# MarbleHE/ABC

Measured on AMD Instinct MI355X. Metric: homomorphic mul+relin/sec, CKKS N=2^14, higher is better.
Workload: dtype u64 (transforms: exact integer arithmetic in f64); 1 GPU; CKKS N=16384, 4 data limbs {50,40,40,40} + special 50-bit prime, ct x ct multiply + relinearize; total_batch=8192, batch_rank0=8192

## Files before the change

### abc_amd/csrc/abc_context.hip

```cpp
#include <cstdlib>
#include <cstring>
#include <mutex>

#include "../../include/abc_hip.h"
#include <dlfcn.h>

#include "abc_context.hpp"
#include "abc_host_math.hpp"

namespace abc {

static thread_local std::string g_err;
void set_error(const std::string &msg) { g_err = msg; }

static bool env_on(const char *name) {
  const char *e = std::getenv(name);
  return e && !(e[0] == '0' && e[1] == 0);
}
void read_switches(abc_hip_ctx *c) {
  abc_hip_ctx::Switches s;
  s.no_fused = env_on("ABC_HIP_NO_FUSED");
  s.no_split = env_on("ABC_HIP_NO_SPLIT");
  s.no_split4 = env_on("ABC_HIP_NO_SPLIT4");
  s.no_isplit = env_on("ABC_HIP_NO_ISPLIT");
  s.no_gsplit = env_on("ABC_HIP_NO_GSPLIT");
  s.no_bsplit = env_on("ABC_HIP_NO_BSPLIT");
  s.no_mixed = env_on("ABC_HIP_NO_MIXED");
  s.no_pack = env_on("ABC_HIP_NO_PACK");
  s.no_key_twin = env_on("ABC_HIP_NO_KEY_TWIN");
  s.no_bmul = env_on("ABC_HIP_NO_BMUL");
  s.no_special8x2 = env_on("ABC_HIP_NO_SPECIAL8X2");
  s.no_bmul_mid = env_on("ABC_HIP_NO_BMUL_MID");
  s.no_finish_lds = env_on("ABC_HIP_NO_FINISH_LDS");
  s.no_iks = env_on("ABC_HIP_NO_IKS");
  s.no_bmul_r6 = env_on("ABC_HIP_NO_BMUL_R6");
  s.no_lean_front = env_on("ABC_HIP_NO_LEAN_FRONT");
  s.no_tensor_intt = env_on("ABC_HIP_NO_TENSOR_INTT");
  s.no_galois_fusion = env_on("ABC_HIP_NO_GALOIS_FUSION");
  if (const char *e = std::getenv("ABC_HIP_CHUNK")) s.chunk = (size_t)std::atol(e);
  if (const char *e = std::getenv("ABC_HIP_FEW_LIMBS")) s.few_limbs = (size_t)std::atol(e);
  if (const char *e = std::getenv("ABC_HIP_LEAN_LIMIT")) s.lean_limit = (size_t)std::atol(e);
  if (const char *e = std::getenv("ABC_HIP_PASS0_TARGET_LIMIT")) s.pass0_target_limit = (size_t)std::atol(e);
  if (const char *e = std::getenv("ABC_HIP_BFV_SCRATCH_MB")) s.bfv_scratch_mb = (size_t)std::atol(e);
  if (const char *e = std::getenv("ABC_HIP_LANE_OFFSET_US")) s.lane_offset_us = (unsigned)std::atoi(e);
  if (const char *e = std::getenv("ABC_HIP_LANES")) {
    s.lanes = std::atoi(e);
    if (s.lanes < 1) s.lanes = 1;
    if (s.lanes > abc_hip_ctx::kMaxLanes) s.lanes = abc_hip_ctx::kMaxLanes;
  }
  c->sw = s;
}

static bool capturing(abc_hip_ctx *c) {
  hipStreamCaptureStatus st = hipStreamCaptureStatusNone;
  if (hipStreamIsCapturing(c->stream, &st) != hipSuccess) return false;
  return st != hipStreamCaptureStatusNone;
}

static int trim_cache(abc_hip_ctx *c) {
  std::lock_guard<std::mutex> lock(c->alloc_mu);
  if (c->free_blocks.empty()) return 0;
  ABC_HIP_CHECK(hipStreamSynchronize(c->stream));
  for (auto &kv : c->free_blocks)
    for (void *p : kv.second) {
      c->block_size.erase(p);
      (void)hipFree(p);
    }
  c->free_blocks.clear();
  c->cached_bytes = 0;
  return 0;
}
static hipError_t malloc_retry(abc_hip_ctx *c, void **p, size_t bytes) {
  hipError_t e = hipMalloc(p, bytes);
  if (e == hipSuccess) return e;
  (void)hipGetLastError();
  if (trim_cache(c)) return e;
  return hipMalloc(p, bytes);
}

void retire_buffer(abc_hip_ctx *c, void *p, uint64_t born) {
  if (!p) return;
  abc_hip_ctx::Held h{p, {}};
  for (auto &kv : c->live_graphs)
    if (kv.second > born) h.graphs.push_back(kv.first);
  if (h.graphs.empty()) {
    (void)hipFree(p);
    return;
  }
  c->held.push_back(std::move(h));
}

int ensure_workspace(abc_hip_ctx *c, size_t bytes) {
  if (bytes <= c->ws_bytes) return 0;
  if (capturing(c)) { set_error("scratch would grow during graph capture: run the sequence once eagerly first"); return 1; }
  if (c->ws) {
    ABC_HIP_CHECK(hipStreamSynchronize(c->stream));
    retire_buffer(c, c->ws, c->ws_born);
    c->ws = nullptr;
    c->ws_bytes = 0;
  }
  size_t want = bytes + bytes / 8;
  ABC_HIP_CHECK(malloc_retry(c, &c->ws, want));
  c->ws_bytes = want;
  c->ws_born = c->graph_seq;
  return 0;
}

int ensure_aux(abc_hip_ctx *c, int which, size_t bytes) {
  if (bytes <= c->aux_bytes[which]) return 0;
  if (capturing(c)) { set_error("scratch would grow during graph capture: run the sequence once eagerly first"); return 1; }
  if (c->aux[which]) {
    ABC_HIP_CHECK(hipStreamSynchronize(c->stream));
    retire_buffer(c, c->aux[which], c->aux_born[which]);
    c->aux[which] = nullptr;
    c->aux_bytes[which] = 0;
  }
  ABC_HIP_CHECK(malloc_retry(c, &c->aux[which], bytes));
  c->aux_bytes[which] = bytes;
  c->aux_born[which] = c->graph_seq;
  return 0;
}
// ... 422 lines not shown
  static const uint64_t p1024[] = {0x7e00001ull};
  static const uint64_t p2048[] = {0x3fffffff000001ull};
  static const uint64_t p4096[] = {0xffffee001ull, 0xffffc4001ull, 0x1ffffe0001ull};
  static const uint64_t p8192[] = {0x7fffffd8001ull, 0x7fffffc8001ull, 0xfffffffc001ull, 0xffffff6c001ull, 0xfffffebc001ull};
  static const uint64_t p16384[] = {0xfffffffd8001ull,  0xfffffffa0001ull,  0xfffffff00001ull,  0x1fffffff68001ull, 0x1fffffff50001ull,
                                    0x1ffffffee8001ull, 0x1ffffffea0001ull, 0x1ffffffe88001ull, 0x1ffffffe48001ull};
  static const uint64_t p32768[] = {0x7fffffffe90001ull, 0x7fffffffbf0001ull, 0x7fffffffbd0001ull, 0x7fffffffba0001ull,
                                    0x7fffffffaa0001ull, 0x7fffffffa50001ull, 0x7fffffff9f0001ull, 0x7fffffff7e0001ull,
                                    0x7fffffff770001ull, 0x7fffffff380001ull, 0x7fffffff330001ull, 0x7fffffff2d0001ull,
                                    0x7fffffff170001ull, 0x7fffffff150001ull, 0x7ffffffef00001ull, 0xfffffffff70001ull};
  const uint64_t *src = nullptr;
  int cnt = 0;
  switch (n) {
    case 1024: src = p1024; cnt = 1; break;
    case 2048: src = p2048; cnt = 1; break;
    case 4096: src = p4096; cnt = 3; break;
    case 8192: src = p8192; cnt = 5; break;
    case 16384: src = p16384; cnt = 9; break;
    case 32768: src = p32768; cnt = 16; break;
    default: set_error("no default BFV coefficient modulus for this ring degree"); return -1;
  }
  for (int i = 0; i < cnt; i++) out[i] = src[i];
  return cnt;
}

uint64_t abc_hip_plain_modulus_batching(size_t n, int bits) {
  try {
    return host::ntt_primes(n, bits, 1)[0];
  } catch (const std::exception &e) {
    set_error(e.what());
    return 0;
  }
}

int abc_hip_create_primes(size_t n, const int *bit_sizes, int count, uint64_t *out) {
  try {
    std::map<int, std::vector<uint64_t>> table;
    for (int i = 0; i < count; i++) table[bit_sizes[i]];
    for (auto &kv : table) {
      size_t need = 0;
      for (int i = 0; i < count; i++) need += (bit_sizes[i] == kv.first);
      kv.second = host::ntt_primes(n, kv.first, need);
    }
    for (int i = 0; i < count; i++) {
      auto &v = table[bit_sizes[i]];
      out[i] = v.back();
      v.pop_back();
    }
    return 0;
  } catch (const std::exception &e) {
    set_error(e.what());
    return 1;
  }
}

int abc_hip_ctx_create(int scheme, int logn, const uint64_t *primes, int nprimes, uint64_t plain_modulus, int device,
                       abc_hip_ctx **out) {
  if (!out) { set_error("null output pointer"); return 1; }
  *out = nullptr;
  if (scheme != ABC_HIP_SCHEME_BFV && scheme != ABC_HIP_SCHEME_CKKS) { set_error("unknown scheme"); return 1; }
  if (logn < 10 || logn > 16) { set_error("logn must be in 10..16"); return 1; }
  if (nprimes < 2 || nprimes > kMaxLimbs) { set_error("need 2..16 primes (data limbs + special prime)"); return 1; }
  const uint64_t two_n = 2ull << logn;
  for (int i = 0; i < nprimes; i++) {
    if (primes[i] >> 60 || !host::is_prime(primes[i]) || primes[i] % two_n != 1) {
      set_error("coefficient modulus primes must be < 2^60, prime and = 1 mod 2N");
      return 1;
    }
    for (int j = 0; j < i; j++)
      if (primes[j] == primes[i]) { set_error("coefficient modulus primes must be distinct"); return 1; }
  }
  if (scheme == ABC_HIP_SCHEME_BFV) {
    if (!host::is_prime(plain_modulus) || plain_modulus % two_n != 1 || plain_modulus >> 32) {
      set_error("plain modulus must be a prime = 1 mod 2N (batching) below 2^32");
      return 1;
    }
  }
  int ndev = 0;
  if (hipGetDeviceCount(&ndev) != hipSuccess || ndev <= 0) { set_error("no HIP device available"); return 1; }
  if (device < 0 || device >= ndev) { set_error("device index out of range"); return 1; }
  if (hipSetDevice(device) != hipSuccess) { set_error("hipSetDevice failed"); return 1; }
  abc_hip_ctx *c = new abc_hip_ctx();
  c->scheme = scheme; c->logn = logn; c->n = 1 << logn; c->K = nprimes; c->L = nprimes - 1; c->device = device;
  c->primes.assign(primes, primes + nprimes);
  c->t = (scheme == ABC_HIP_SCHEME_BFV) ? plain_modulus : 0;
  int rc = 1;
  try {
    rc = build_context(c);
  } catch (const std::exception &e) {
    set_error(e.what());
  }
  if (!rc && hipStreamCreateWithFlags(&c->own_stream, hipStreamNonBlocking) != hipSuccess) {
    set_error("hipStreamCreate failed");
    rc = 1;
  }
  if (!rc) c->stream = c->own_stream;
  if (!rc && (hipEventCreate(&c->ev0) != hipSuccess || hipEventCreate(&c->ev1) != hipSuccess ||
              hipEventCreateWithFlags(&c->lane_fork, hipEventDisableTiming) != hipSuccess)) {
    set_error("hipEventCreate failed");
    rc = 1;
  }
  int mask_mod = 0;
  if (const char *e = std::getenv("ABC_HIP_CU_MASK")) mask_mod = std::atoi(e);
  for (int i = 0; !rc && i < abc_hip_ctx::kMaxLanes; i++) {
    hipError_t se;
    if (mask_mod >= 2) {
      uint32_t mask[8];
      for (int w = 0; w < 8; w++) {
        mask[w] = 0;
        for (int b = 0; b < 32; b++)
          if (((w * 32 + b) % mask_mod) == (i % mask_mod)) mask[w] |= 1u << b;
      }
      se = hipExtStreamCreateWithCUMask(&c->lane[i], 8, mask);
    } else {
      se = hipStreamCreateWithFlags(&c->lane[i], hipStreamNonBlocking);
    }
    if (hipEventCreateWithFlags(&c->lane_join[i], hipEventDisableTiming) != hipSuccess || se != hipSuccess) {
      set_error("lane stream / event creation failed");
      rc = 1;
    }
  }
  if (!rc && !env_on("ABC_HIP_SYNC_ALLOC")) {
    c->cache_alloc = true;
    size_t free_b = 0, total_b = 0;
    if (hipMemGetInfo(&free_b, &total_b) == hipSuccess) c->cache_cap = total_b / 4;
  }
  if (rc) { abc_hip_ctx_destroy(c); return 1; }
  *out = c;
  return 0;
}

void abc_hip_ctx_destroy(abc_hip_ctx *c) {
  if (!c) return;
  (void)hipSetDevice(c->device);
  (void)hipDeviceSynchronize();
  (void)hipFree(c->d_mods); (void)hipFree(c->d_tw); (void)hipFree(c->d_ftw); (void)hipFree(c->d_cst); (void)hipFree(c->d_cstf);
  (void)hipFree(c->d_slot_map);
  (void)hipFree(c->d_ckks_codec);
  drop_key_twins(c, nullptr);
  (void)hipFree(c->d_sk); (void)hipFree(c->d_pk); (void)hipFree(c->d_relin);
  for (auto &kv : c->d_galois) (void)hipFree(kv.second);
  (void)hipFree(c->ws);
  for (void *p : c->aux) (void)hipFree(p);
  for (auto &h : c->held) (void)hipFree(h.p);
  for (auto &kv : c->block_size) (void)hipFree(kv.first);
  if (c->own_stream) (void)hipStreamDestroy(c->own_stream);
  if (c->ev0) (void)hipEventDestroy(c->ev0);
  if (c->ev1) (void)hipEventDestroy(c->ev1);
  if (c->lane_fork) (void)hipEventDestroy(c->lane_fork);
  for (int i = 0; i < abc_hip_ctx::kMaxLanes; i++) {
    if (c->lane_join[i]) (void)hipEventDestroy(c->lane_join[i]);
    if (c->lane[i]) (void)hipStreamDestroy(c->lane[i]);
  }
  delete c;
}

int abc_hip_ctx_info(const abc_hip_ctx *c, int what) {
  if (!c) return -1;
  switch (what) {
    case 0: return c->scheme;
    case 1: return c->logn;
    case 2: return c->K;
    case 3: return c->L;
    case 4: return c->device;
    case 5: return c->nBsk;
    case 6: return (int)c->held.size();
// ... 471 lines not shown
```

### abc_amd/csrc/abc_context.hpp

```cpp
#pragma once

#include <hip/hip_runtime.h>

#include <map>
#include <mutex>
#include <unordered_map>
#include <string>
#include <vector>

#include "abc_modarith.hpp"
#include "abc_ntt.hpp"

namespace abc {

constexpr int kMaxLimbs = 16;

struct LimbMap {
  int id[kMaxLimbs + 1];
};

struct DevConst {
  u64 inv_special[kMaxLimbs], inv_special_s[kMaxLimbs];
  u64 inv_qlast[kMaxLimbs][kMaxLimbs], inv_qlast_s[kMaxLimbs][kMaxLimbs];
  u64 special_mod_q[kMaxLimbs], special_mod_q_s[kMaxLimbs];
  double inv_special_c[kMaxLimbs], inv_special_cq[kMaxLimbs];
  double special_c[kMaxLimbs], special_cq[kMaxLimbs];
  double inv_qlast_c[kMaxLimbs][kMaxLimbs], inv_qlast_cq[kMaxLimbs][kMaxLimbs];
  u64 q_mod_t, upper_half_threshold, t;
  u64 coeff_div_plain[kMaxLimbs], upper_half_increment[kMaxLimbs];
  int nq, nB, nBsk, pad_;
  u64 mtilde_mod_q[kMaxLimbs];
  u64 inv_punct_q[kMaxLimbs];
  u64 q_to_bsk[kMaxLimbs][kMaxLimbs];
  u64 q_to_mtilde[kMaxLimbs];
  u64 neg_inv_q_mod_mtilde;
  u64 q_mod_bsk[kMaxLimbs], inv_mtilde_mod_bsk[kMaxLimbs], inv_q_mod_bsk[kMaxLimbs];
  u64 inv_punct_B[kMaxLimbs];
  u64 B_to_q[kMaxLimbs][kMaxLimbs];
  u64 B_to_msk[kMaxLimbs];
  u64 inv_B_mod_msk, B_mod_q[kMaxLimbs];
  u64 t_mod_q[kMaxLimbs], t_mod_bsk[kMaxLimbs];
  u64 ext_q[kMaxLimbs], ext_q_s[kMaxLimbs];
  u64 flr_q[kMaxLimbs], flr_q_s[kMaxLimbs];
  u64 tinvq_bsk[kMaxLimbs], tinvq_bsk_s[kMaxLimbs];
  u64 inv_q_mod_bsk_s[kMaxLimbs], inv_mtilde_mod_bsk_s[kMaxLimbs], inv_punct_B_s[kMaxLimbs];
  u64 inv_B_mod_msk_s, B_mod_q_s[kMaxLimbs];
  u64 dec_q[kMaxLimbs], dec_q_s[kMaxLimbs];
  u64 q_to_bsk_s[kMaxLimbs][kMaxLimbs], B_to_q_s[kMaxLimbs][kMaxLimbs], B_to_msk_s[kMaxLimbs], q_mod_bsk_s[kMaxLimbs];
  u64 tgamma_mod_q[kMaxLimbs], q_to_t[kMaxLimbs], q_to_gamma[kMaxLimbs];
  u64 neg_inv_q_mod_t, neg_inv_q_mod_gamma, inv_gamma_mod_t, gamma;
};

struct DevConstFp {
  double ext_q[kMaxLimbs][2], flr_q[kMaxLimbs][2], B_mod_q[kMaxLimbs][2];
  double q_to_bsk[kMaxLimbs][kMaxLimbs][2];
  double B_to_q[kMaxLimbs][kMaxLimbs][2];
  double q_mod_bsk[kMaxLimbs][2], inv_mtilde_mod_bsk[kMaxLimbs][2], tinvq_bsk[kMaxLimbs][2], inv_q_mod_bsk[kMaxLimbs][2];
  double inv_punct_B[kMaxLimbs][2], B_to_msk[kMaxLimbs][2], inv_B_mod_msk[2];
};

struct DevCtx {
  const Mod *mods;
  const u64 *tw;
  const double *ftw;
  const DevConst *cst;
  const DevConstFp *cstf;
  const u32 *slot_map;
  int logn, n;
  int ps;
  int K, L;
  int id_bsk, id_t, id_gamma, id_mtilde;
};

__device__ __forceinline__ NttTable ntt_table(const DevCtx &c, int mid) {
  const u64 *b = c.tw + (size_t)mid * 4 * c.n;
  NttTable t;
  t.tw = reinterpret_cast<const u64x2 *>(b);
  t.itw = reinterpret_cast<const u64x2 *>(b + 2 * (size_t)c.n);
  return t;
}

__device__ __forceinline__ Mod mod_at(const DevCtx &c, int id) {
  const ABC_CONST_AS Mod *p = (const ABC_CONST_AS Mod *)(c.mods + id);
  Mod m;
  m.q = p->q; m.mu = p->mu; m.two_q = p->two_q; m.shift = p->shift; m.bits = p->bits;
  m.inv_n = p->inv_n; m.inv_n_s = p->inv_n_s; m.qd = p->qd; m.qinv = p->qinv;
  m.inv_n_c = p->inv_n_c; m.inv_n_cq = p->inv_n_cq;
  return m;
}
__device__ __forceinline__ FpTable fp_table(const DevCtx &c, int mid) {
  const double *b = c.ftw + (size_t)mid * 4 * c.n;
  FpTable t;
  t.tw = (const ABC_CONST_AS f64x2 *)(b);
  t.itw = (const ABC_CONST_AS f64x2 *)(b + 2 * (size_t)c.n);
  return t;
}

}

struct abc_hip_ctx {
  int scheme = 0, logn = 0, n = 0, K = 0, L = 0, device = 0;
  std::vector<uint64_t> primes;
  uint64_t t = 0;
  hipStream_t stream = nullptr;
  hipStream_t own_stream = nullptr;
  hipEvent_t ev0 = nullptr, ev1 = nullptr;
  static constexpr int kMaxLanes = 4;
  hipStream_t lane[kMaxLanes] = {nullptr, nullptr, nullptr, nullptr};
  hipEvent_t lane_fork = nullptr, lane_join[kMaxLanes] = {nullptr, nullptr, nullptr, nullptr};
  std::vector<abc::Mod> h_mods;
  std::vector<uint64_t> mod_values;
  int nB = 0, nBsk = 0;
  abc::DevCtx dc{};
  abc::DevConst h_cst{};
  abc::Mod *d_mods = nullptr;
  uint64_t *d_tw = nullptr;
  double *d_ftw = nullptr;
  bool cache_alloc = false;
  std::mutex alloc_mu;
  size_t cached_bytes = 0, cache_cap = (size_t)8 << 30;
  std::unordered_map<size_t, std::vector<void *>> free_blocks;
  std::unordered_map<void *, size_t> block_size;
  bool capture_active = false;
  std::unordered_map<void *, std::vector<void *>> pin;
  std::unordered_map<void *, bool> parked;
  std::unordered_map<size_t, std::vector<void *>> cap_free;
  std::unordered_map<void *, bool> cap_born;
  bool behz_fp = false;
  bool use_fp = true;
  struct Switches {
    bool no_fused = false, no_split = false, no_split4 = false, no_isplit = false, no_gsplit = false, no_lean_front = false, no_bsplit = false, no_mixed = false, no_pack = false, no_key_twin = false, no_special8x2 = false, no_bmul = false, no_bmul_mid = false, no_finish_lds = false, no_iks = false, no_bmul_r6 = false, no_tensor_intt = false;
    bool no_galois_fusion = false;
    size_t chunk = 0, few_limbs = 48, lean_limit = 96, bfv_scratch_mb = 0, pass0_target_limit = 128;
    int lanes = 2;
    unsigned lane_offset_us = 0;
  } sw;
  abc::DevConst *d_cst = nullptr;
  abc::DevConstFp *d_cstf = nullptr;
  uint32_t *d_slot_map = nullptr;
  void *d_ckks_codec = nullptr;
  uint64_t *d_sk = nullptr, *d_pk = nullptr, *d_relin = nullptr;
  std::map<uint32_t, uint64_t *> d_galois;
  std::unordered_map<const uint64_t *, double *> key_twins;
  std::unordered_map<const uint64_t *, uint64_t *> key_shoups;
  std::vector<uint32_t> galois_order;
  void *ws = nullptr;
  size_t ws_bytes = 0;
  void *aux[3] = {nullptr, nullptr, nullptr};
  size_t aux_bytes[3] = {0, 0, 0};
  uint64_t graph_seq = 0;
  std::unordered_map<void *, uint64_t> live_graphs;
  struct Held {
    void *p;
    std::vector<void *> graphs;
  };
  std::vector<Held> held;
  uint64_t ws_born = 0, aux_born[3] = {0, 0, 0};
  size_t limb_words() const { return (size_t)n; }
  size_t key_words() const { return (size_t)L * 2 * K * n; }
};

namespace abc {

void set_error(const std::string &msg);
#define ABC_HIP_CHECK(expr)                                                                         \
  do {                                                                                              \
    hipError_t e_ = (expr);                                                                         \
    if (e_ != hipSuccess) {                                                                         \
      abc::set_error(std::string(#expr) + ": " + hipGetErrorString(e_));                            \
      return 1;                                                                                     \
    }                                                                                               \
  } while (0)

int ensure_workspace(abc_hip_ctx *c, size_t bytes);
int ensure_aux(abc_hip_ctx *c, int which, size_t bytes);
void retire_buffer(abc_hip_ctx *c, void *p, uint64_t born);
void read_switches(abc_hip_ctx *c);

LimbMap key_limb_map(const abc_hip_ctx *c, int nl);
int launch_ntt_fwd(abc_hip_ctx *c, u64 *d, const LimbMap &map, int nl, size_t total_limbs);
int launch_ks_expand_ntt_fp(abc_hip_ctx *c, const u64 *tcoef, size_t tstride, u64 *dec, const LimbMap &map, int nl, size_t count);
int launch_ntt_fwd_from2(abc_hip_ctx *c, const u64 *src, const u64 *src2, u64 *d, const LimbMap &map, int nl, size_t total_limbs);
int launch_ntt_fwd_from(abc_hip_ctx *c, const u64 *src, u64 *d, const LimbMap &map, int nl, size_t total_limbs);
int launch_ntt_inv(abc_hip_ctx *c, u64 *d, const LimbMap &map, int nl, size_t total_limbs);
int launch_ntt_inv_strided_part(abc_hip_ctx *c, u64 *d, const LimbMap &map, int nl, size_t total_limbs, bool integer_only = false);
int big_block_log(void);

int launch_addsub(abc_hip_ctx *c, const u64 *a, const u64 *b, u64 *out, int nl, size_t polys, int op);
int launch_ckks_tensor(abc_hip_ctx *c, const u64 *a, const u64 *b, u64 *out3, int nl, size_t count);
int keyswitch_generic(abc_hip_ctx *c, const u64 *target, size_t target_stride, const u64 *key, u64 *out2, int nl,
                      size_t count, const u64 *addend, size_t addend_stride, bool add_c1, u32 ginv = 0);
int launch_ks_tmod(abc_hip_ctx *c, const u64 *prodS, u64 *tmod, int nl, size_t polys);
int launch_ks_finish(abc_hip_ctx *c, const u64 *prodD, const u64 *tmod, u64 *out, const u64 *addend, size_t addend_stride,
                     bool add_c1, int nl, size_t count);
int launch_galois(abc_hip_ctx *c, const u64 *in, u64 *out, int nl, size_t polys, uint32_t elt, bool ntt_form);
int launch_rescale(abc_hip_ctx *c, const u64 *in, u64 *out, int size, int nl, size_t count);
int launch_drop_last(abc_hip_ctx *c, const u64 *in, u64 *out, int size, int nl, size_t count);

int bfv_multiply(abc_hip_ctx *c, const u64 *a, const u64 *b, u64 *out3, size_t count);
int bfv_multiply_plain(abc_hip_ctx *c, const u64 *ct, const u64 *plain, size_t plain_stride, u64 *out, int size, size_t count);
int bfv_addsub_plain(abc_hip_ctx *c, const u64 *ct, const u64 *plain, size_t plain_stride, u64 *out, int size, size_t count, int sub);
int ckks_multiply_plain(abc_hip_ctx *c, const u64 *ct, const u64 *plain, size_t plain_stride, u64 *out, int size, int nl, size_t count);
int ckks_add_plain(abc_hip_ctx *c, const u64 *ct, const u64 *plain, size_t plain_stride, u64 *out, int size, int nl, size_t count, int sub);
int batch_encode(abc_hip_ctx *c, const int64_t *values, u64 *plain, size_t count);
int batch_decode(abc_hip_ctx *c, const u64 *plain, int64_t *values, size_t count);
int ckks_encode(abc_hip_ctx *c, const double *re, const double *im, size_t values_per_row, double scale, int nl, u64 *plain,
                size_t count);
int ckks_decode(abc_hip_ctx *c, const u64 *plain, int nl, double scale, double *re, double *im, size_t count);
int encrypt(abc_hip_ctx *c, const u64 *plain, uint64_t seed, u64 *ct, size_t count);
int decrypt(abc_hip_ctx *c, const u64 *ct, int size, int nl, u64 *plain, size_t count);
int keygen(abc_hip_ctx *c, uint64_t seed);
int keygen_secure(abc_hip_ctx *c);
int encrypt_secure(abc_hip_ctx *c, const u64 *plain, u64 *ct, size_t count);
int microbench(abc_hip_ctx *c, int which, int iters, double *ms);

int rotate_fused(abc_hip_ctx *c, const u64 *in, u32 elt, const u64 *key, u64 *out, int nl, size_t count);
int keyswitch_fused(abc_hip_ctx *c, const u64 *target, size_t target_stride, const u64 *key, u64 *out2, int nl, size_t count,
                    const u64 *addend, size_t addend_stride, bool add_c1);
int ckks_mul_relin_fused(abc_hip_ctx *c, const u64 *a, const u64 *b, u64 *out, int nl, size_t count);
bool gsplit_applies(const abc_hip_ctx *c, int nl);
size_t gsplit_scratch_words(const abc_hip_ctx *c, int nl);
int gsplit_chunk15(abc_hip_ctx *c, hipStream_t st, u64 *scratch, size_t cc, int nl, int mode, const u64 *opa, const u64 *opb,
                   size_t opa_stride, size_t opb_stride, int add_c1, const u64 *key, u64 *out, u32 gelt);
void gsplit_front14(hipStream_t st, abc_hip_ctx *c, size_t cc, int nl, int mode, const u64 *opa, const u64 *opb, size_t opa_stride,
                    double *hinv, double *part, u32 gelt, int pack = 0);
bool split4_main_subset(hipStream_t st, abc_hip_ctx *c, size_t cc, int nl, int mode, const double *part, const double *tpart, const u64 *opa,
                        const u64 *opb, size_t opa_stride, size_t opb_stride, int add_c1, const u64 *key, u64 *out, u32 gelt, u32 imap,
                        int ni);
bool gsplit_main_subset15(hipStream_t st, abc_hip_ctx *c, size_t cc, int nl, int mode, const double *part, const double *tpart, const u64 *opa,
                          const u64 *opb, size_t opa_stride, size_t opb_stride, int add_c1, const u64 *key, u64 *out, u32 gelt, u32 imap,
                          int ni);
void gsplit_main_deep_subset15(hipStream_t st, abc_hip_ctx *c, size_t cc, int nl, int mode, const double *part, const double *tpart,
                               const u64 *opa, const u64 *opb, size_t opa_stride, size_t opb_stride, int add_c1, const u64 *key, u64 *out,
                               u32 gelt, u64 imap, int ni);
bool bsplit_applies(const abc_hip_ctx *c, int nl);
bool bsplit_big_applies(const abc_hip_ctx *c, int nl);
bool iks_bfv_applies(const abc_hip_ctx *c, int nl);
int bsplit_big(abc_hip_ctx *c, const u64 *target, size_t target_stride, const u64 *key, u64 *out, int nl, size_t count, const u64 *addend,
               size_t addend_stride, bool add_c1, u32 ginv = 0);
int bsplit_back14(abc_hip_ctx *c, hipStream_t st, size_t cc, int nl, const double *part, double *half, const u64 *key, const u64 *addend,
                  size_t addend_stride, int add_c1, u64 *out, u32 ginv = 0);
int bsplit_back13(abc_hip_ctx *c, hipStream_t st, size_t cc, int nl, const double *part, double *half, const u64 *key, const u64 *addend,
                  size_t addend_stride, int add_c1, u64 *out, u32 ginv = 0);
const double *key_twin(abc_hip_ctx *c, const u64 *key);
const double *key_twin_lookup(const abc_hip_ctx *c, const u64 *key);
void drop_key_twins(abc_hip_ctx *c, const u64 *key );
void refresh_key_twins(abc_hip_ctx *c, const u64 *key );
void refresh_key_shoups(abc_hip_ctx *c, const u64 *key );
void release_key(abc_hip_ctx *c, u64 *key);
int fork_lanes(abc_hip_ctx *c, int lanes);
int join_lanes(abc_hip_ctx *c, int lanes);
struct LaneScope {
  abc_hip_ctx *c;
  int lanes;
  bool forked = false;
  LaneScope(abc_hip_ctx *c_, int lanes_) : c(c_), lanes(lanes_) {}
  int fork() {
    if (fork_lanes(c, lanes)) return 1;
    forked = true;
    return 0;
  }
  int join() {
    forked = false;
    return join_lanes(c, lanes);
  }
  ~LaneScope() {
    if (forked) (void)join_lanes(c, lanes);
  }
};

bool bmul_applies(const abc_hip_ctx *c);
bool bmul_multiply_applies(const abc_hip_ctx *c);
int launch_ntt_fwd_block_part(abc_hip_ctx *c, u64 *d, const LimbMap &map, int nl, size_t total_limbs);
int launch_bfv_tensor_inv_block(abc_hip_ctx *c, const u64 *a, const u64 *b, size_t ct_stride, u64 *d, const LimbMap &map, int nlm,
                                size_t count);
int bmul_split(abc_hip_ctx *c, const u64 *a, const u64 *b, u64 *out, size_t count, bool relin);
bool isplit_applies(const abc_hip_ctx *c, int nl);
size_t isplit_scratch_words(const abc_hip_ctx *c, int nl);
int isplit_chunk(abc_hip_ctx *c, hipStream_t st, u64 *scratch, size_t cc, int nl, int mode, const u64 *opa, const u64 *opb,
                 size_t opa_stride, size_t opb_stride, int add_c1, const u64 *key, u64 *out, u32 gelt);

}
```

### abc_amd/csrc/abc_kernels_fused.hip

```cpp
#include <type_traits>

#include "abc_context.hpp"
#include "abc_host_math.hpp"

namespace abc {

static inline unsigned stream_grid(size_t items, int block) {
  size_t g = (items + block - 1) / block;
  const size_t cap = 256 * 8 * 4;
  return (unsigned)(g < cap ? (g ? g : 1) : cap);
}

template <int LB>
__global__ __launch_bounds__((1 << LB) / 16) void k_fused_tensor_intt(DevCtx c, const u64 *__restrict__ a,
                                                                      const u64 *__restrict__ b, u64 *__restrict__ c01,
                                                                      u64 *__restrict__ c2coef, u64 *__restrict__ c2ntt, int nl) {
  __shared__ u64 lds[lds_words(LB)];
  const int j = blockIdx.x % nl;
  const size_t ct = blockIdx.x / nl;
  const size_t N = (size_t)1 << LB, pw = (size_t)nl * N;
  const Mod m = c.mods[j];
  const NttTable t = ntt_table(c, j);
  const u64 *__restrict__ a0 = a + ct * 2 * pw + j * N, *__restrict__ a1 = a0 + pw;
  const u64 *__restrict__ b0 = b + ct * 2 * pw + j * N, *__restrict__ b1 = b0 + pw;
// ... 949 lines not shown
            x[k] = fp_mulmod(x1[k], y1[k], q, qinv);
            d0[k] = fp_mulmod(x0[k], y0[k], q, qinv);
            d1[k] = fp_mulmod(x0[k], y1[k], q, qinv) + fp_mulmod(x1[k], y0[k], q, qinv);
          }
        } else {
#pragma unroll
          for (int k = 0; k < 2; k++) {
            x[k] = fp_from_u64(o.xs[k]);
            d0[k] = fp_from_u64(o.d0s[k]);
            d1[k] = fp_from_u64(o.d1s[k]);
          }
        }
      } else {
        const int w = Jx < I ? Jx : Jx - 1;
        const f64x2 v = *reinterpret_cast<const f64x2 *>(dyn + w * lds_words(10) + lds_pad(e));
        x[0] = v.x;
        x[1] = v.y;
      }
      s0[0] += fp_mulmod(x[0], kd(o.k0[Jx].x), q, qinv);
      s0[1] += fp_mulmod(x[1], kd(o.k0[Jx].y), q, qinv);
      s1[0] += fp_mulmod(x[0], kd(o.k1[Jx].x), q, qinv);
      s1[1] += fp_mulmod(x[1], kd(o.k1[Jx].y), q, qinv);
      if (Jx == 7) {
#pragma unroll
        for (int k = 0; k < 2; k++) {
          s0[k] = fp_centre(s0[k], q, qinv);
          s1[k] = fp_centre(s1[k], q, qinv);
        }
      }
    }
    const f64x2 u0 = *reinterpret_cast<const f64x2 *>(tt0 + lds_pad(e)), u1 = *reinterpret_cast<const f64x2 *>(tt1 + lds_pad(e));
    u64x2 r;
    r.x = fp_to_canon(fp_mul_lazy(s0[0] - u0.x, inv, inv_q, q) + d0[0], q, qinv);
    r.y = fp_to_canon(fp_mul_lazy(s0[1] - u0.y, inv, inv_q, q) + d0[1], q, qinv);
    *reinterpret_cast<u64x2 *>(out + ((ct * 2 + 0) * nl + I) * N + base + e) = r;
    r.x = fp_to_canon(fp_mul_lazy(s1[0] - u1.x, inv, inv_q, q) + d1[0], q, qinv);
    r.y = fp_to_canon(fp_mul_lazy(s1[1] - u1.y, inv, inv_q, q) + d1[1], q, qinv);
    *reinterpret_cast<u64x2 *>(out + ((ct * 2 + 1) * nl + I) * N + base + e) = r;
  };
  if (keyf) compute_pair(2 * (int)threadIdx.x, ops, std::true_type{});
  else compute_pair(2 * (int)threadIdx.x, ops, std::false_type{});
}

template <int MODE, bool GAL>
static bool launch_split4_main(hipStream_t st, abc_hip_ctx *c, size_t cc, int nl, const double *part, const double *tpart, const u64 *opa,
                               const u64 *opb, size_t opa_stride, size_t opb_stride, int add_c1, const u64 *key, u64 *out, u32 gelt,
                               u32 imap = 0x76543210u, int ni = -1, int pack = 0) {
  if (nl < 1 || nl > 7) return false;
  if (ni < 0) ni = nl;
  if (ni == 0) return true;
  const dim3 grid((unsigned)(cc * ni * 16)), block(512);
  const size_t lds = (size_t)((nl + 1) * lds_words(10)) * 8 + 1024 * 16;
#define ABC_TM4(NLV)                                                                                                                 \
  hipLaunchKernelGGL((k_split4_main_fp<MODE, GAL, NLV>), grid, block, lds, st, c->dc, part, tpart, opa, opb, opa_stride, opb_stride, \
                     add_c1, key, out, gelt, imap, ni, pack, keyf)
  const double *keyf = key_twin_lookup(c, key);
  switch (nl) {
    case 1: ABC_TM4(1); break;
    case 2: ABC_TM4(2); break;
    case 3: ABC_TM4(3); break;
    case 4: ABC_TM4(4); break;
    case 5: ABC_TM4(5); break;
    case 6: ABC_TM4(6); break;
    default: ABC_TM4(7); break;
  }
#undef ABC_TM4
  return true;
}
bool split4_main_subset(hipStream_t st, abc_hip_ctx *c, size_t cc, int nl, int mode, const double *part, const double *tpart, const u64 *opa,
                        const u64 *opb, size_t opa_stride, size_t opb_stride, int add_c1, const u64 *key, u64 *out, u32 gelt, u32 imap,
                        int ni) {
  if (mode == 0) return launch_split4_main<0, false>(st, c, cc, nl, part, tpart, opa, opb, opa_stride, opb_stride, add_c1, key, out, gelt, imap, ni);
  if (gelt) return launch_split4_main<1, true>(st, c, cc, nl, part, tpart, opa, opb, opa_stride, opb_stride, add_c1, key, out, gelt, imap, ni);
  return launch_split4_main<1, false>(st, c, cc, nl, part, tpart, opa, opb, opa_stride, opb_stride, add_c1, key, out, gelt, imap, ni);
}


template <int MODE, bool GAL>
static void launch_split3(hipStream_t st, abc_hip_ctx *c, const FusedScratch &s, size_t cc, int nl, const u64 *opa, const u64 *opb,
                          size_t opa_stride, size_t opb_stride, int add_c1, const u64 *key, u64 *out, u32 gelt, int pack) {
  launch_split_special(st, c, cc, nl, (const double *)s.dec, key, (double *)s.tsp);
  hipLaunchKernelGGL(k_split3_pass_fp<14>, dim3((unsigned)(cc * 2 * 4)), dim3(256), 0, st, c->dc, (const double *)s.tsp, (double *)s.ksacc,
                     nl, pack);
  if (!c->sw.no_split4 && nl <= 5 && launch_split4_main<MODE, GAL>(st, c, cc, nl, (const double *)s.dec, (const double *)s.ksacc, opa, opb,
                                                        opa_stride, opb_stride, add_c1, key, out, gelt, 0x76543210u, -1, pack))
    return;
  launch_split3_main<MODE, GAL>(st, c, cc, nl, (const double *)s.dec, (const double *)s.ksacc, opa, opb, opa_stride, opb_stride, add_c1,
                                key, out, gelt);
}

static inline int pack_half_done(const abc_hip_ctx *c, int nl) {
  return (!c->sw.no_pack && !c->sw.no_split4 && nl >= 1 && nl <= 5) ? 1 : 0;
}
static inline bool all_fp(const abc_hip_ctx *c) {
  bool fp = c->use_fp;
  for (int j = 0; j < c->K; j++) fp = fp && fp_ok(c->h_mods[j].bits);
  return fp;
}
static inline bool needs_guard(const abc_hip_ctx *c) {
  bool guard = false;
  for (int j = 0; j < c->K; j++) guard = guard || !unguarded_ok(c->h_mods[j].bits);
  return guard;
}

template <int LB>
static int keyswitch_stage(abc_hip_ctx *c, hipStream_t st, const FusedScratch &s, const u64 *coef, size_t coef_stride, const u64 *ntt,
                           size_t ntt_stride, const u64 *key, const u64 *addend, size_t addend_stride, bool add_c1, u64 *out, int nl,
                           size_t cc, int dec_ready = 0 ) {
  const size_t N = (size_t)1 << LB;
  const dim3 block((1 << LB) / 16);
  const bool ckks = (c->scheme == 2);
  const bool guard = needs_guard(c);
  const unsigned g2a = (unsigned)(cc * (nl + 1) * nl);
  const unsigned g3 = (unsigned)(cc * 2 * nl);
  if (all_fp(c)) {
    if (!dec_ready)
      hipLaunchKernelGGL(k_fused_ks_decomp_ntt_fp<LB>, dim3(g2a), block, 0, st, c->dc, coef, coef_stride, s.dec, nl, ckks ? 1 : 0);
    hipLaunchKernelGGL(k_fused_ks_mac, dim3(stream_grid(cc * (nl + 1) * (N / 2), 256)), dim3(256), 0, st, c->dc, s.dec,
                       ckks ? ntt : (const u64 *)nullptr, ntt_stride, key, s.ksacc, s.tsp, nl, cc);
    hipLaunchKernelGGL(k_fused_ks_special_intt_fp<LB>, dim3((unsigned)(cc * 2)), block, 0, st, c->dc, s.tsp, s.tlast);
    if (ckks)
      hipLaunchKernelGGL((k_fused_ks_moddown_fp<LB, false>), dim3(g3), block, 0, st, c->dc, s.ksacc, s.tlast, addend, addend_stride,
                         add_c1 ? 1 : 0, out, nl, (int)(cc * 2), 0u);
    else
      hipLaunchKernelGGL(k_fused_ks_moddown_bfv_fp<LB>, dim3(g3), block, 0, st, c->dc, s.ksacc, s.tlast, addend, addend_stride,
                         add_c1 ? 1 : 0, out, nl);
    ABC_HIP_CHECK(hipGetLastError());
    return 0;
  }
  bool lazy = !guard;
  for (int j = 0; j < c->K; j++) lazy = lazy && c->h_mods[j].bits <= 55;
  if (guard)
    hipLaunchKernelGGL((k_fused_ks_decomp_ntt<LB, true, false>), dim3(g2a), block, 0, st, c->dc, coef, coef_stride, s.dec, nl,
                       ckks ? 1 : 0);
  else if (lazy)
    hipLaunchKernelGGL((k_fused_ks_decomp_ntt<LB, false, true>), dim3(g2a), block, 0, st, c->dc, coef, coef_stride, s.dec, nl,
                       ckks ? 1 : 0);
  else
    hipLaunchKernelGGL((k_fused_ks_decomp_ntt<LB, false, false>), dim3(g2a), block, 0, st, c->dc, coef, coef_stride, s.dec, nl,
                       ckks ? 1 : 0);
  hipLaunchKernelGGL(k_fused_ks_mac, dim3(stream_grid(cc * (nl + 1) * (N / 2), 256)), dim3(256), 0, st, c->dc, s.dec,
                     ckks ? ntt : (const u64 *)nullptr, ntt_stride, key, s.ksacc, s.tsp, nl, cc);
  hipLaunchKernelGGL(k_fused_ks_special_intt<LB>, dim3((unsigned)(cc * 2)), block, 0, st, c->dc, s.tsp, s.tlast);
  if (!ckks)
    hipLaunchKernelGGL(k_fused_ks_moddown_bfv<LB>, dim3(g3), block, 0, st, c->dc, s.ksacc, s.tlast, addend, addend_stride,
                       add_c1 ? 1 : 0, out, nl);
  else if (guard)
    hipLaunchKernelGGL((k_fused_ks_moddown<LB, true>), dim3(g3), block, 0, st, c->dc, s.ksacc, s.tlast, addend, addend_stride,
                       add_c1 ? 1 : 0, out, nl);
  else
    hipLaunchKernelGGL((k_fused_ks_moddown<LB, false>), dim3(g3), block, 0, st, c->dc, s.ksacc, s.tlast, addend, addend_stride,
                       add_c1 ? 1 : 0, out, nl);
  ABC_HIP_CHECK(hipGetLastError());
  return 0;
}

struct ChunkPlan {
  size_t chunk;
  int lanes;
};
static ChunkPlan plan_chunks(const abc_hip_ctx *c, int nl, size_t count) {
  ChunkPlan p{c->sw.chunk, c->sw.lanes};
  if (count <= 8) p.lanes = 1;
  if (!p.chunk) {
    const size_t per_ct_bytes = fused_scratch_limbs(nl) * c->n * 8;
    const size_t cap = ((size_t)4 << 30) / per_ct_bytes / (size_t)p.lanes;
// ... 280 lines not shown
```

Baseline: 409,800 mul+relin/s.

## Add persistent split5 main kernel streaming ciphertexts with LDS DMA prefetch

Adds a new keyswitch main kernel that keeps each block resident across a run of ciphertexts. It holds the relin key limbs in registers and double-buffers the next ciphertext's partial data into LDS through global_load_lds while computing the current one. The run length is sized from the CU count so the grid roughly fills the device. The aim is to cut repeated key and twiddle loads and to overlap memory fetch with the NTT tail and tensor product. The cost is high register and LDS pressure, with only 2-4 blocks per CU, plus hand-written waitcnt sequencing that may be fragile.

```diff
diff --git a/abc_amd/csrc/abc_context.hip b/abc_amd/csrc/abc_context.hip
--- a/abc_amd/csrc/abc_context.hip
+++ b/abc_amd/csrc/abc_context.hip
@@ -37,6 +37,8 @@
   s.no_lean_front = env_on("ABC_HIP_NO_LEAN_FRONT");
   s.no_tensor_intt = env_on("ABC_HIP_NO_TENSOR_INTT");
   s.no_galois_fusion = env_on("ABC_HIP_NO_GALOIS_FUSION");
+  s.no_stream_main = env_on("ABC_HIP_NO_STREAM_MAIN");
+  if (const char *e = std::getenv("ABC_HIP_MAIN_RUN")) s.main_run = (size_t)std::atol(e);
   if (const char *e = std::getenv("ABC_HIP_CHUNK")) s.chunk = (size_t)std::atol(e);
   if (const char *e = std::getenv("ABC_HIP_FEW_LIMBS")) s.few_limbs = (size_t)std::atol(e);
   if (const char *e = std::getenv("ABC_HIP_LEAN_LIMIT")) s.lean_limit = (size_t)std::atol(e);
@@ -625,6 +627,7 @@
   if (hipSetDevice(device) != hipSuccess) { set_error("hipSetDevice failed"); return 1; }
   abc_hip_ctx *c = new abc_hip_ctx();
   c->scheme = scheme; c->logn = logn; c->n = 1 << logn; c->K = nprimes; c->L = nprimes - 1; c->device = device;
+  if (hipDeviceGetAttribute(&c->cus, hipDeviceAttributeMultiprocessorCount, device) != hipSuccess) c->cus = 0;
   c->primes.assign(primes, primes + nprimes);
   c->t = (scheme == ABC_HIP_SCHEME_BFV) ? plain_modulus : 0;
   int rc = 1;
diff --git a/abc_amd/csrc/abc_context.hpp b/abc_amd/csrc/abc_context.hpp
--- a/abc_amd/csrc/abc_context.hpp
+++ b/abc_amd/csrc/abc_context.hpp
@@ -100,6 +100,7 @@
 
 struct abc_hip_ctx {
   int scheme = 0, logn = 0, n = 0, K = 0, L = 0, device = 0;
+  int cus = 0;
   std::vector<uint64_t> primes;
   uint64_t t = 0;
   hipStream_t stream = nullptr;
@@ -131,6 +132,8 @@
   struct Switches {
     bool no_fused = false, no_split = false, no_split4 = false, no_isplit = false, no_gsplit = false, no_lean_front = false, no_bsplit = false, no_mixed = false, no_pack = false, no_key_twin = false, no_special8x2 = false, no_bmul = false, no_bmul_mid = false, no_finish_lds = false, no_iks = false, no_bmul_r6 = false, no_tensor_intt = false;
     bool no_galois_fusion = false;
+    bool no_stream_main = false;
+    size_t main_run = 0;
     size_t chunk = 0, few_limbs = 48, lean_limit = 96, bfv_scratch_mb = 0, pass0_target_limit = 128;
     int lanes = 2;
     unsigned lane_offset_us = 0;
@@ -224,6 +227,8 @@
                    size_t opa_stride, size_t opb_stride, int add_c1, const u64 *key, u64 *out, u32 gelt);
 void gsplit_front14(hipStream_t st, abc_hip_ctx *c, size_t cc, int nl, int mode, const u64 *opa, const u64 *opb, size_t opa_stride,
                     double *hinv, double *part, u32 gelt, int pack = 0);
+bool launch_split5_main(hipStream_t st, abc_hip_ctx *c, size_t cc, int nl, const double *part, const double *tpart, const u64 *opa,
+                        const u64 *opb, const u64 *key, u64 *out, int pack);
 bool split4_main_subset(hipStream_t st, abc_hip_ctx *c, size_t cc, int nl, int mode, const double *part, const double *tpart, const u64 *opa,
                         const u64 *opb, size_t opa_stride, size_t opb_stride, int add_c1, const u64 *key, u64 *out, u32 gelt, u32 imap,
                         int ni);
diff --git a/abc_amd/csrc/abc_kernels_fused.hip b/abc_amd/csrc/abc_kernels_fused.hip
--- a/abc_amd/csrc/abc_kernels_fused.hip
+++ b/abc_amd/csrc/abc_kernels_fused.hip
@@ -1055,6 +1055,9 @@
   launch_split_special(st, c, cc, nl, (const double *)s.dec, key, (double *)s.tsp);
   hipLaunchKernelGGL(k_split3_pass_fp<14>, dim3((unsigned)(cc * 2 * 4)), dim3(256), 0, st, c->dc, (const double *)s.tsp, (double *)s.ksacc,
                      nl, pack);
+  if (MODE == 0 && !c->sw.no_split4 && !c->sw.no_stream_main &&
+      launch_split5_main(st, c, cc, nl, (const double *)s.dec, (const double *)s.ksacc, opa, opb, key, out, pack))
+    return;
   if (!c->sw.no_split4 && nl <= 5 && launch_split4_main<MODE, GAL>(st, c, cc, nl, (const double *)s.dec, (const double *)s.ksacc, opa, opb,
                                                         opa_stride, opb_stride, add_c1, key, out, gelt, 0x76543210u, -1, pack))
     return;
diff --git a/abc_amd/csrc/abc_kernels_split5.hip b/abc_amd/csrc/abc_kernels_split5.hip
--- /dev/null
+++ b/abc_amd/csrc/abc_kernels_split5.hip
@@ -0,0 +1,209 @@
+#include <type_traits>
+
+#include "abc_context.hpp"
+#include "abc_host_math.hpp"
+
+namespace abc {
+
+static __device__ __forceinline__ double fp_mulmod(double x, double y, double q, double qinv) {
+  const double h = x * y;
+  const double l = __builtin_fma(x, y, -h);
+  const double c = __builtin_rint(h * qinv);
+  return __builtin_fma(-c, q, h) + l;
+}
+
+__device__ __forceinline__ void lds_dma16(const void *g, void *lds) {
+  __builtin_amdgcn_global_load_lds(g, (__attribute__((address_space(3))) void *)lds, 16, 0, 0);
+}
+
+template <int NL>
+__global__ __launch_bounds__(512, NL <= 4 ? 4 : 2) void k_split5_main_fp(DevCtx c, const double *__restrict__ part,
+                                                                   const double *__restrict__ tpart, const u64 *__restrict__ opa,
+                                                                   const u64 *__restrict__ opb, const u64 *__restrict__ key,
+                                                                   u64 *__restrict__ out, int pack, const double *__restrict__ keyf,
+                                                                   unsigned cc, unsigned run) {
+  extern __shared__ double dyn[];
+  static_assert(NL + 1 <= 8, "one wavefront per limb, eight wavefronts");
+  constexpr int nl = NL, NT = 512, PER = 2;
+  const int W = __builtin_amdgcn_readfirstlane((int)(threadIdx.x >> 6));
+  const int lane = threadIdx.x & 63;
+  const int e = 2 * (int)threadIdx.x;
+  const u32 voff = (u32)e * 8;
+  const int blk = blockIdx.x & 15;
+  const int I = (int)((blockIdx.x >> 4) % (unsigned)nl);
+  const unsigned ct0 = ((blockIdx.x >> 4) / (unsigned)nl) * run, ct1 = ct0 + run < cc ? ct0 + run : cc;
+  const size_t N = (size_t)c.n, base = (size_t)blk << 10;
+  const Mod m = mod_at(c, I);
+  const FpTable t = fp_table(c, I);
+  const double q = m.qd, qinv = m.qinv;
+  f64x2 *ltw = reinterpret_cast<f64x2 *>(dyn + (nl + 1) * lds_words(10));
+  const size_t pw = (size_t)nl * N;
+  const ABC_CONST_AS DevConst *cst = (const ABC_CONST_AS DevConst *)c.cst;
+  const double inv = cst->inv_special_c[I], inv_q = cst->inv_special_cq[I];
+  const bool has_limb = W <= nl;
+  const int Wc = has_limb ? W : 0;
+  const double *__restrict__ src0 = (Wc < nl - 1) ? part + ((size_t)I * nl + (Wc < I ? Wc : Wc + 1)) * (size_t)c.ps + base
+                                                  : tpart + ((size_t)(Wc - (nl - 1)) * nl + I) * (size_t)c.ps + base;
+  const size_t sstride = ((Wc < nl - 1) ? (size_t)(nl + 1) * nl : (size_t)2 * nl) * (size_t)c.ps;
+  const int pk = pack ? pack_kind(m.bits) : 0;
+  double *buf = dyn + Wc * lds_words(10);
+  const u32 loff = (u32)lane * 16;
+  auto at = [](const void *p, u32 off) { return (const void *)(reinterpret_cast<const unsigned char *>(p) + off); };
+  auto stage = [&](unsigned ct) {
+    const double *s = src0 + ct * sstride;
+    if (pk == 0) {
+#pragma unroll
+      for (int k = 0; k < 8; k++) lds_dma16(at(s + (k << 7), loff), buf + (k << 7));
+    } else {
+      const u32 *lo = reinterpret_cast<const u32 *>(s - base) + base;
+      const unsigned char *hi = reinterpret_cast<const unsigned char *>(s - base) + 4 * N + (pk == 1 ? base : 2 * base);
+#pragma unroll
+      for (int k = 0; k < 4; k++)
+        lds_dma16(at(lo + (k << 8), loff), reinterpret_cast<u32 *>(buf) + (k << 8));
+      lds_dma16(at(hi, loff), reinterpret_cast<unsigned char *>(buf) + 4096);
+      if (pk == 2) lds_dma16(at(hi + 1024, loff), reinterpret_cast<unsigned char *>(buf) + 5120);
+    }
+  };
+
+  {
+    f64x2 twv[PER];
+    block_twiddles_fetch<10, f64x2, PER>(t.tw, 4, blk, (int)threadIdx.x, NT, twv);
+    block_twiddles_store<10, f64x2, PER>(ltw, (int)threadIdx.x, NT, twv);
+  }
+  __syncthreads();
+  f64x2 kd0[NL], kd1[NL];
+  {
+    const double *kw = keyf ? keyf : reinterpret_cast<const double *>(key);
+#pragma unroll
+    for (int Jx = 0; Jx < NL; Jx++) {
+      kd0[Jx] = *reinterpret_cast<const f64x2 *>(at(kw + (((size_t)Jx * 2 + 0) * c.K + I) * N + base, voff));
+      kd1[Jx] = *reinterpret_cast<const f64x2 *>(at(kw + (((size_t)Jx * 2 + 1) * c.K + I) * N + base, voff));
+    }
+    if (!keyf) {
+      auto cv = [](double w) { return fp_from_u64((u64)__double_as_longlong(w)); };
+#pragma unroll
+      for (int Jx = 0; Jx < NL; Jx++) {
+        kd0[Jx].x = cv(kd0[Jx].x); kd0[Jx].y = cv(kd0[Jx].y);
+        kd1[Jx].x = cv(kd1[Jx].x); kd1[Jx].y = cv(kd1[Jx].y);
+      }
+    }
+  }
+  if (has_limb) stage(ct0);
+
+  for (unsigned ct = ct0; ct < ct1; ct++) {
+    if (has_limb) {
+      if (ct == ct0) __builtin_amdgcn_s_waitcnt(0x0F70);
+      else __builtin_amdgcn_s_waitcnt(0x0F72);
+    }
+    const u64 *pa = opa + ct * 2 * pw + (size_t)I * N + base, *pb = opb + ct * 2 * pw + (size_t)I * N + base;
+    const u64x2 a0 = *reinterpret_cast<const u64x2 *>(at(pa, voff)), a1 = *reinterpret_cast<const u64x2 *>(at(pa + pw, voff));
+    const u64x2 b0 = *reinterpret_cast<const u64x2 *>(at(pb, voff)), b1 = *reinterpret_cast<const u64x2 *>(at(pb + pw, voff));
+
+    const int ln = __builtin_amdgcn_update_dpp(0, lane, 0xE4, 0xF, 0xF, false);
+    const int el = 2 * (int)(threadIdx.x & ~63u) + 2 * ln;
+    if (has_limb) {
+      double xin[16];
+      if (pk == 0) {
+#pragma unroll
+        for (int k = 0; k < 8; k++) {
+          const f64x2 v = *reinterpret_cast<const f64x2 *>(buf + (k << 7) + 2 * ln);
+          xin[k] = v.x;
+          xin[8 + k] = v.y;
+        }
+      } else if (pk == 1) {
+#pragma unroll
+        for (int k = 0; k < 8; k++) {
+          const int i = (k << 7) + 2 * ln;
+          u64x2 r;
+          r.x = *reinterpret_cast<const u64 *>(reinterpret_cast<const u32 *>(buf) + i);
+          r.y = *reinterpret_cast<const unsigned short *>(reinterpret_cast<const unsigned char *>(buf) + 4096 + i);
+          pack_decode_pair<1>(r, xin[k], xin[8 + k]);
+        }
+      } else {
+#pragma unroll
+        for (int k = 0; k < 8; k++) {
+          const int i = (k << 7) + 2 * ln;
+          u64x2 r;
+          r.x = *reinterpret_cast<const u64 *>(reinterpret_cast<const u32 *>(buf) + i);
+          r.y = *reinterpret_cast<const u32 *>(reinterpret_cast<const unsigned char *>(buf) + 4096 + 2 * i);
+          pack_decode_pair<2>(r, xin[k], xin[8 + k]);
+        }
+      }
+      if (m.bits >= 49) {
+#pragma unroll
+        for (int r = 0; r < 16; r++) xin[r] = fp_centre(xin[r], q, qinv);
+      }
+      ntt_fwd_tail1024_pairs<FpTail>(buf, xin, [&](int, int i, double v) { buf[lds_pad(i)] = v; }, t, m, 4, blk, ln, ltw);
+    }
+    __syncthreads();
+    f64x2 lx[NL];
+#pragma unroll
+    for (int Jx = 0; Jx < NL; Jx++) {
+      const int w = Jx < I ? Jx : Jx > I ? Jx - 1 : 0;
+      lx[Jx] = *reinterpret_cast<const f64x2 *>(dyn + w * lds_words(10) + lds_pad(el));
+    }
+    const f64x2 u0 = *reinterpret_cast<const f64x2 *>(dyn + (nl - 1) * lds_words(10) + lds_pad(el));
+    const f64x2 u1 = *reinterpret_cast<const f64x2 *>(dyn + nl * lds_words(10) + lds_pad(el));
+    __builtin_amdgcn_s_waitcnt(0x0F70);
+    __syncthreads();
+    if (has_limb && ct + 1 < ct1) stage(ct + 1);
+
+    {
+      double s0[2] = {0.0, 0.0}, s1[2] = {0.0, 0.0}, d0[2] = {0.0, 0.0}, d1[2] = {0.0, 0.0};
+#pragma unroll
+      for (int Jx = 0; Jx < NL; Jx++) {
+        double x[2] = {lx[Jx].x, lx[Jx].y};
+        if (Jx == I) {
+          const double x0[2] = {fp_from_u64(a0.x), fp_from_u64(a0.y)}, x1[2] = {fp_from_u64(a1.x), fp_from_u64(a1.y)};
+          const double y0[2] = {fp_from_u64(b0.x), fp_from_u64(b0.y)}, y1[2] = {fp_from_u64(b1.x), fp_from_u64(b1.y)};
+#pragma unroll
+          for (int k = 0; k < 2; k++) {
+            x[k] = fp_mulmod(x1[k], y1[k], q, qinv);
+            d0[k] = fp_mulmod(x0[k], y0[k], q, qinv);
+            d1[k] = fp_mulmod(x0[k], y1[k], q, qinv) + fp_mulmod(x1[k], y0[k], q, qinv);
+          }
+        }
+        s0[0] += fp_mulmod(x[0], kd0[Jx].x, q, qinv);
+        s0[1] += fp_mulmod(x[1], kd0[Jx].y, q, qinv);
+        s1[0] += fp_mulmod(x[0], kd1[Jx].x, q, qinv);
+        s1[1] += fp_mulmod(x[1], kd1[Jx].y, q, qinv);
+      }
+      u64x2 r;
+      r.x = fp_to_canon(fp_mul_lazy(s0[0] - u0.x, inv, inv_q, q) + d0[0], q, qinv);
+      r.y = fp_to_canon(fp_mul_lazy(s0[1] - u0.y, inv, inv_q, q) + d0[1], q, qinv);
+      *reinterpret_cast<u64x2 *>(const_cast<void *>(at(out + ((ct * 2 + 0) * (size_t)nl + I) * N + base, voff))) = r;
+      r.x = fp_to_canon(fp_mul_lazy(s1[0] - u1.x, inv, inv_q, q) + d1[0], q, qinv);
+      r.y = fp_to_canon(fp_mul_lazy(s1[1] - u1.y, inv, inv_q, q) + d1[1], q, qinv);
+      *reinterpret_cast<u64x2 *>(const_cast<void *>(at(out + ((ct * 2 + 1) * (size_t)nl + I) * N + base, voff))) = r;
+    }
+  }
+}
+
+static unsigned split5_run(const abc_hip_ctx *c, size_t cc, int nl) {
+  if (c->sw.main_run) return (unsigned)(c->sw.main_run < cc ? c->sw.main_run : cc);
+  const size_t target = 2 * (size_t)(c->cus > 0 ? c->cus : 256), slots = (size_t)nl * 16;
+  size_t r = (cc * slots + target - 1) / target;
+  return (unsigned)(r < 1 ? 1 : r > cc ? cc : r);
+}
+
+bool launch_split5_main(hipStream_t st, abc_hip_ctx *c, size_t cc, int nl, const double *part, const double *tpart, const u64 *opa,
+                               const u64 *opb, const u64 *key, u64 *out, int pack) {
+  if (nl < 1 || nl > 5 || cc == 0) return false;
+  const unsigned run = split5_run(c, cc, nl);
+  const dim3 grid((unsigned)((cc + run - 1) / run * nl * 16)), block(512);
+  const size_t lds = (size_t)((nl + 1) * lds_words(10)) * 8 + 1024 * 16;
+  const double *keyf = key_twin_lookup(c, key);
+#define ABC_TM5(NLV) \
+  hipLaunchKernelGGL((k_split5_main_fp<NLV>), grid, block, lds, st, c->dc, part, tpart, opa, opb, key, out, pack, keyf, (unsigned)cc, run)
+  switch (nl) {
+    case 1: ABC_TM5(1); break;
+    case 2: ABC_TM5(2); break;
+    case 3: ABC_TM5(3); break;
+    case 4: ABC_TM5(4); break;
+    default: ABC_TM5(5); break;
+  }
+#undef ABC_TM5
+  return true;
+}
+
+}
```

Result: no change. 411,200 mul+relin/s, median of 6 (+0.3%).
